# TritonDataCenter/dragnet

Measured on NVIDIA B200. Metric: json_records_per_sec, higher is better.
Workload: dtype u8

## Files before the change

dragnet_b200/csrc/api.cu:

```cuda
#include <cuda_runtime.h>
#include <dlfcn.h>
#include <fcntl.h>
#include <sys/stat.h>
#include <unistd.h>

#include <algorithm>
#include <map>
#include <condition_variable>
#include <mutex>
#include <thread>
#include <cerrno>
#include <cmath>
#include <cstdio>
#include <cstdlib>
#include <cstring>
#include <string>
#include <vector>

#include "../../include/dragnet_gpu.h"
#include "plan.h"
#include "result.h"
#include "scan_kernel.cuh"
#include "fast_kernel.cuh"
#include "jit.h"
// ... 114 lines not shown
	size_t ring_cap = 0;
	u8 *d_ring[RING_SLOTS] = {};
	u8 *h_stage[RING_SLOTS] = {};
	cudaEvent_t ev_ready[RING_SLOTS] = {}, ev_free[RING_SLOTS] = {};
	bool slot_used[RING_SLOTS] = {};
	size_t next_slot = 0;
	u8 *d_carry = nullptr;
	size_t carry_len = 0;
	u8 *d_side = nullptr;
	u8 *file_buf = nullptr;
	cudaEvent_t file_done[32] = {};
	std::vector<std::pair<cudaEvent_t, cudaEvent_t>> ev_pairs;
	std::vector<cudaEvent_t> ev_pool;
	double kernel_ms = 0;
	uint64_t launches = 0, kernel_bytes = 0, bytes_fed = 0;
	uint64_t aux_launches = 0;
	cudaEvent_t ev_init = nullptr;
	bool finished = false;
	bool tmpl_enabled = true, tmpl_tried = false;
	bool warp_kernel = false;
	u32 wslice = DNG_W_SLICE_MAX;
	int kernel_pref = 0;
	u32 w_sslots = 0, w_s1slots = 0;
	unsigned long long *h_live = nullptr;
	unsigned long long learn_lines = 0, learn_tmpl = 0;
	unsigned long long seen_lines = 0, seen_long = 0;
	int relearns = 0;
	u8 *d_tmpl = nullptr;
	u32 tmpl_bytes = 0, ntemplates = 0;
	FPlan fplan;
	FPlan *d_fplan = nullptr;
	u8 *d_ftmpl = nullptr;
	u32 ftmpl_bytes = 0, nftemplates = 0, ftmpl_leaf_off = 0, ftmpl_pool_off = 0;
	bool f_kernel = false;
	u32 f_nt = DNG_F_NT;
	unsigned long long seen_over = 0, seen_aggr = 0;
	bool f_probed = false;
	u32 f_nsl = 13;
	double mean_line = 224;
	u32 f_smem_max = 0;
	int jit_mode = 1;
	std::shared_ptr<JitKernels> jit;
	uint64_t jit_launches = 0;
	MissEnt *d_miss = nullptr;
	u32 *d_miss_n = nullptr;
	u32 miss_cap = 0;
	unsigned long long seen_tmpl = 0;
	std::string err;
	int err_code = 0;

	int fail(int code, const std::string &m) {
		if (!err_code) {
			err_code = code;
			err = m;
		}
		return code;
	}
	int cuda(cudaError_t e, const char *what) {
		if (e == cudaSuccess)
			return 0;
		return fail(DNG_ECUDA, std::string(what) + ": " +
		    cudaGetErrorString(e));
	}
};

#define CK(s, call) do { if ((s)->cuda((call), #call)) return (s)->err_code; } while (0)
// ... 17 lines not shown
__global__ void resolve_pairs_kernel(const DevPlan *plan, const u8 *lines,
    const u32 *se, u32 n, TResolved *out)
{
	u32 i = blockIdx.x * blockDim.x + threadIdx.x;
	if (i >= n)
		return;
	RecState R;
	parse_record(lines + se[2 * i], se[2 * i + 1] - se[2 * i], *plan, R);
	out[i].flags = R.flags;
	out[i].set_mask = R.set_mask;
	for (int k = 0; k < MAX_SLOTS; k++)
		out[i].slots[k] = ((R.set_mask >> k) & 1) ? R.slots[k] : 0;
}

static std::mutex g_fnt_mu;
static std::map<unsigned long long, u32> g_fnt_memo;

static unsigned long long fplan_hash(const FPlan &F)
{
	unsigned long long h = 1469598103934665603ull;
	const u8 *p = (const u8 *)&F;
	for (size_t i = 0; i < sizeof (F); i++)
		h = (h ^ p[i]) * 1099511628211ull;
	return h;
}

static void fnt_remember(const dng_scan *s)
{
	std::lock_guard<std::mutex> g(g_fnt_mu);
	g_fnt_memo[fplan_hash(s->fplan)] = s->f_nt;
}

int learn_ftemplates(dng_scan *s, const std::vector<TCandidate> &cands,
    const std::vector<TResolved> &res, size_t sampled_lines)
{
	std::vector<TResolved> fres(res.size());
	for (size_t i = 0; i < res.size(); i++)
		fplan_resolve(s->plan.dev, res[i], fres[i]);
	std::vector<u8> blob, accepted;
	u32 nt = 0;
	tmpl_build(cands, fres, TMPL_RESERVE, blob, &nt, true, &accepted);
	cached_free(s->d_ftmpl);
	s->d_ftmpl = nullptr;
	s->ftmpl_bytes = 0;
	s->nftemplates = 0;
	if (!blob.empty()) {
		const THdr *th = (const THdr *)blob.data();
		s->ftmpl_leaf_off = th->leaf_off;
		s->ftmpl_pool_off = th->pool_off;
	}
	size_t covered = 0;
	for (size_t i = 0; i < cands.size(); i++)
		if (accepted[i])
			covered += cands[i].count;
	if (!blob.empty()) {
		size_t padded = (blob.size() + 127) & ~(size_t)127;
		blob.resize(padded, 0);
		CK(s, DEV_ALLOC(s, &s->d_ftmpl, padded));
		CK(s, cudaMemcpyAsync(s->d_ftmpl, blob.data(), padded,
		    cudaMemcpyHostToDevice, s->stream));
		CK(s, cudaStreamSynchronize(s->stream));
		s->ftmpl_bytes = (u32)padded;
		s->nftemplates = nt;
	}
	s->jit.reset();
	if (s->jit_mode && !blob.empty())
		s->jit = jit_request(jit_source(blob.data(), blob.size(), &s->fplan),
		    (int)s->f_nsl, s->device, (int)s->f_smem_max,
		    s->jit_mode == 2);
	if (s->kernel_pref == 0)
		s->f_kernel = s->warp_kernel && !blob.empty() &&
		    covered * 10 >= sampled_lines * 9 &&
		    s->mean_line * DNG_F_NLCAP >= 32.0 * 16 * s->f_nsl * 1.5;
	return 0;
}

int learn_templates(dng_scan *s, const u8 *data, unsigned long long start,
    unsigned long long nbytes)
{
	s->tmpl_tried = true;
	if (!s->tmpl_enabled && s->kernel_pref != 0)
		return 0;
	size_t n = (size_t)std::min<unsigned long long>(nbytes - start,
	    TMPL_SAMPLE_BYTES);
	u8 *hbuf = nullptr;
	CK(s, HOST_ALLOC(&hbuf, TMPL_SAMPLE_BYTES));
	struct Release {
		u8 *p;
		~Release() { cached_free(p); }
	} release{hbuf};
	CK(s, cudaMemcpyAsync(hbuf, data + start, n, cudaMemcpyDeviceToHost,
	    s->stream));
	CK(s, cudaStreamSynchronize(s->stream));
	struct { u8 *p; u8 *data() const { return p; }
	    u8 operator[](size_t i) const { return p[i]; } } head{hbuf};
	if (s->kernel_pref == 0) {
		size_t longest = 0, run = 0;
		for (size_t i = 0; i < n; i++) {
			if (head[i] == '\n') {
				longest = std::max(longest, run);
				run = 0;
			} else {
// ... 53 lines not shown
	    (size_t)TMPL_MAX_LEAVES * (TMPL_MAX_LINE + 1) + 16);
	if (e == cudaSuccess)
		e = DEV_ALLOC(s, &d_offs, 2 * (TMPL_MAX_LEAVES + 1) * sizeof (u32));
	if (e == cudaSuccess)
		e = DEV_ALLOC(s, &d_res, TMPL_MAX_LEAVES * sizeof (TResolved));
	if (e == cudaSuccess)
		e = cudaMemcpyAsync(d_lines, lines.data(), lines.size(),
		    cudaMemcpyHostToDevice, s->stream);
	std::vector<u32> se;
	for (size_t i = 0; i < cands.size(); i++) {
		se.push_back(offs[i]);
		se.push_back(offs[i + 1] - 1);
	}
	if (e == cudaSuccess)
		e = cudaMemcpyAsync(d_offs, se.data(), se.size() * sizeof (u32),
		    cudaMemcpyHostToDevice, s->stream);
	if (e == cudaSuccess) {
		s->aux_launches++;
		resolve_pairs_kernel<<<1, 32, 0, s->stream>>>(s->d_plan, d_lines,
		    d_offs, (u32)cands.size(), d_res);
		e = cudaGetLastError();
	}
	if (e == cudaSuccess)
		e = cudaMemcpyAsync(res.data(), d_res,
		    res.size() * sizeof (TResolved), cudaMemcpyDeviceToHost,
		    s->stream);
	if (e == cudaSuccess)
		e = cudaStreamSynchronize(s->stream);
	cached_free(d_lines);
	cached_free(d_offs);
	cached_free(d_res);
	if (e != cudaSuccess)
		return s->cuda(e, "template resolve");
	if (s->fplan.ok && learn_ftemplates(s, cands, res, sampled_lines))
		return s->err_code;
	std::vector<u8> blob;
	u32 nt = 0;
	tmpl_build(cands, res, TMPL_RESERVE, blob, &nt);
	if (blob.empty())
		return 0;
	size_t padded = (blob.size() + 127) & ~(size_t)127;
	blob.resize(padded, 0);
	cached_free(s->d_tmpl);
	s->d_tmpl = nullptr;
	s->tmpl_bytes = 0;
	CK(s, DEV_ALLOC(s, &s->d_tmpl, padded));
	CK(s, cudaMemcpyAsync(s->d_tmpl, blob.data(), padded,
	    cudaMemcpyHostToDevice, s->stream));
	CK(s, cudaStreamSynchronize(s->stream));
	s->tmpl_bytes = (u32)padded;
	s->ntemplates = nt;
	return 0;
}

template <int NSL>
void launch_fkernel(dng_scan *s, const FScanArgs &a, u32 grid)
{
	scan_kernel_f<NSL><<<grid, s->f_nt, fkernel_smem<NSL>(a.tmpl_bytes,
	    a.s1slots, a.sslots, a.nrows, s->f_nt / 32), s->stream>>>(a);
}

template <int NSL>
void fkernel_slots(const dng_scan *s, u32 nrows, u32 tmpl_room, u32 *s1, u32 *s2)
{
	const size_t fixed = fkernel_smem<NSL>(tmpl_room, 0, 0, nrows,
	    s->f_nt / 32);
	const size_t room = s->f_smem_max > fixed ? s->f_smem_max - fixed : 0;
	u32 n1 = 32;
	while (n1 < 1024 && (size_t)n1 * 2 * sizeof (SSlot1) +
	    DNG_SSLOTS_MIN * sizeof (SSlot) <= room * 3 / 4)
		n1 *= 2;
	const size_t left = room - std::min(room, (size_t)n1 * sizeof (SSlot1));
	u32 n2 = DNG_SSLOTS_MIN;
	while (n2 * 2 <= DNG_SSLOTS_MAX && (size_t)n2 * 2 * sizeof (SSlot) <= left)
		n2 *= 2;
	*s1 = n1;
	*s2 = n2;
}

int launch_fscan(dng_scan *s, const u8 *data, unsigned long long start,
    unsigned long long nbytes, bool final)
{
	if (!s->d_miss) {
		s->miss_cap = (u32)env_size("DNG_MISS_CAP", (size_t)4 << 20);
		CK(s, DEV_ALLOC(s, &s->d_miss, (size_t)s->miss_cap *
		    sizeof (MissEnt)));
		CK(s, DEV_ALLOC(s, &s->d_miss_n, 64));
		CK(s, cudaMemsetAsync(s->d_miss_n, 0, 64, s->stream));
	}
	const unsigned long long skip = start & ~15ull;
	data += skip;
	start -= skip;
	nbytes -= skip;
	FScanArgs a;
	a.data = data;
	a.start = start;
	a.nbytes = nbytes;
	a.fplan = s->d_fplan;
	a.plan = s->d_plan;
	a.tmpl = s->d_ftmpl;
	a.tmpl_bytes = s->ftmpl_bytes;
	a.leaf_off = s->ftmpl_leaf_off;
	a.pool_off = s->ftmpl_pool_off;
	a.counters = s->d_counters;
	a.tab = s->tab;
	a.final = final ? 1 : 0;
	a.nrows = s->fplan.nrows;
	a.miss = s->d_miss;
	a.miss_cap = s->miss_cap;
	a.miss_n = s->d_miss_n;
	const u32 nsl = s->f_nsl;
	const unsigned long long chunk = 32ull * 16 * nsl;
	a.nchunks = (u32)((nbytes + chunk - 1) / chunk);
	const u32 nw = s->f_nt / 32;
	const u32 grid = std::min<u32>((a.nchunks + nw - 1) / nw,
	    (u32)s->sm_count);
	const u32 nwarps = grid * nw;
	a.seg = std::max<u32>(1, std::min<u32>(DNG_F_SEG,
	    a.nchunks / (nwarps * 8)));
	a.seg_next = s->d_miss_n + 1;
	cudaMemsetAsync(s->d_miss_n, 0, 2 * sizeof (u32), s->stream);
	cudaEvent_t e0 = get_event(s), e1 = get_event(s);
	cudaEventRecord(e0, s->stream);
	const bool jit = s->jit && s->jit->state.load() == 1 && s->ftmpl_bytes;
	const u32 tmpl_room = jit ? 0 : (u32)TMPL_RESERVE;
	if (jit)
		a.tmpl_bytes = 0;
	size_t smem = 0;
	switch (nsl) {
	case 7:
		fkernel_slots<7>(s, a.nrows, tmpl_room, &a.s1slots, &a.sslots);
		smem = fkernel_smem<7>(a.tmpl_bytes, a.s1slots, a.sslots, a.nrows,
		    s->f_nt / 32);
		if (!jit)
			launch_fkernel<7>(s, a, grid);
		break;
	case 9:
		fkernel_slots<9>(s, a.nrows, tmpl_room, &a.s1slots, &a.sslots);
		smem = fkernel_smem<9>(a.tmpl_bytes, a.s1slots, a.sslots, a.nrows,
		    s->f_nt / 32);
		if (!jit)
			launch_fkernel<9>(s, a, grid);
		break;
	case 11:
		fkernel_slots<11>(s, a.nrows, tmpl_room, &a.s1slots, &a.sslots);
		smem = fkernel_smem<11>(a.tmpl_bytes, a.s1slots, a.sslots, a.nrows,
		    s->f_nt / 32);
		if (!jit)
			launch_fkernel<11>(s, a, grid);
		break;
	default:
		fkernel_slots<13>(s, a.nrows, tmpl_room, &a.s1slots, &a.sslots);
		smem = fkernel_smem<13>(a.tmpl_bytes, a.s1slots, a.sslots, a.nrows,
		    s->f_nt / 32);
		if (!jit)
			launch_fkernel<13>(s, a, grid);
		break;
	}
	cudaError_t le = cudaSuccess;
	if (jit) {
		void *args[] = { &a };
		le = cudaLaunchKernel((const void *)s->jit->kern, dim3(grid),
		    dim3(s->f_nt), args, smem, s->stream);
		s->jit_launches++;
	}
	if (le == cudaSuccess)
		le = cudaGetLastError();
	FMissArgs ma;
	ma.data = data;
	ma.start = start;
	ma.plan = s->d_plan;
	ma.plan_bytes = s->plan_bytes;
	ma.counters = s->d_counters;
	ma.tab = s->tab;
	ma.s1slots = 64;
	ma.sslots = 1024;
	ma.miss = s->d_miss;
	ma.miss_n = s->d_miss_n;
	ma.miss_cap = s->miss_cap;
	if (le == cudaSuccess) {
		scan_miss_kernel<<<s->sm_count * 2, DNG_MISS_NT, s->plan_bytes +
		    ma.s1slots * sizeof (SSlot1) + ma.sslots * sizeof (SSlot),
		    s->stream>>>(ma);
		le = cudaGetLastError();
	}
	cudaEventRecord(e1, s->stream);
	if (!s->h_live && HOST_ALLOC(&s->h_live, NCTR * sizeof (unsigned long long))
// ... 1069 lines not shown
	if (!s)
		return;
	cudaSetDevice(s->device);
	if (s->stream)
		cudaStreamSynchronize(s->stream);
	if (s->own_stream && s->own_stream != s->stream)
		cudaStreamSynchronize(s->own_stream);
	if (s->copy_stream)
		cudaStreamSynchronize(s->copy_stream);
	drain_events(s);
	if (s->ev_init)
		cudaEventDestroy(s->ev_init);
	for (auto e : s->ev_pool)
		cudaEventDestroy(e);
	for (size_t i = 0; i < RING_SLOTS; i++) {
		if (s->d_ring[i]) {
			cached_free(s->d_ring[i]);
			cudaEventDestroy(s->ev_ready[i]);
			cudaEventDestroy(s->ev_free[i]);
		}
		if (s->h_stage[i])
			cached_free(s->h_stage[i]);
	}
	if (s->file_buf) {
		cached_free(s->file_buf);
		for (int i = 0; i < 32; i++)
			cudaEventDestroy(s->file_done[i]);
	}
	cached_free(s->h_live);
	cached_free(s->d_plan);
	cached_free(s->d_tmpl);
	cached_free(s->d_fplan);
	cached_free(s->d_ftmpl);
	cached_free(s->d_miss);
	cached_free(s->d_miss_n);
	cached_free(s->tab.entries);
	cached_free(s->tab.arena);
	cached_free(s->tab.misc);
	cached_free(s->d_counters);
	cached_free(s->d_nl);
	cached_free(s->d_carry);
	cached_free(s->d_side);
	if (s->own_stream)
		cudaStreamDestroy(s->own_stream);
	if (s->copy_stream)
		cudaStreamDestroy(s->copy_stream);
	delete s;
}

void *dng_pinned_alloc(size_t len)
{
	void *p = nullptr;
	if (cudaMallocHost(&p, len) != cudaSuccess)
		return nullptr;
	return p;
}

void dng_pinned_free(void *p)
{
	if (p)
		cudaFreeHost(p);
}


size_t dng_result_count(const dng_result *r)
{
// ... 188 lines not shown
```

dragnet_b200/csrc/fast.cuh:

```cuda
#ifndef DNG_FAST_CUH
#define DNG_FAST_CUH

#include "fast.h"
#include "tmpl.cuh"

#ifdef DNG_JIT_HOT
#define DNG_PLAN_LOOP _Pragma("unroll")
#else
#define DNG_PLAN_LOOP _Pragma("unroll 1")
#endif

namespace dng {

#include "fscan.cuh"

DNG_HD u32 fcap_off(u32 c) { return c & 0xfff; }
DNG_HD u32 fcap_len(u32 c) { return (c >> 12) & 0xfff; }
DNG_HD u32 fcap_type(u32 c) { return (c >> 24) & 7; }
DNG_HD u32 fcap_flag(u32 c) { return c >> 27; }

template <class M>
DNG_HD bool fmatch(M &m, u32 len, bool active, u32 &defmask)
{
	u32 p = 0;
// ... 461 lines not shown
		if (n > 1)
			first |= fpiece_byte(m, F, pc, 1) << 24;
		const u32 fm = n >= 2 ? ~0u : n == 1 ? 0x00ffffffu : 0x0000ffffu;
		diff |= (kc.next() ^ first) & fm;
		if (n > 2) {
			if (pc.kind == 0) {
				FWords<M> ws(m, F, pc, 2);
				const u32 r = n - 2;
#pragma unroll 1
				for (u32 i = 0; i < r; i += 4) {
					const u32 mk = i + 4 <= r ? ~0u :
					    (1u << (8 * (r & 3))) - 1;
					diff |= (kc.next() ^ ws.next()) & mk;
				}
			} else {
				const u32 r = n - 2;
#pragma unroll 1
				for (u32 i = 0; i < r; i += 4) {
					u32 w = 0;
					for (u32 x = 0; x < 4 && i + x < r; x++)
						w |= fpiece_byte(m, F, pc, 2 + i + x)
						    << (8 * x);
					const u32 mk = i + 4 <= r ? ~0u :
					    (1u << (8 * (r & 3))) - 1;
					diff |= (kc.next() ^ w) & mk;
				}
			}
		}
		o += 2 + n;
	}
	return diff == 0;
}

template <class M>
DNG_HD void fkey_write(M &m, const FPlan &F, u32 defmask, u8 *out)
{
	u32 o = 0;
DNG_PLAN_LOOP
	for (u32 j = 0; j < F.ncols; j++) {
		FPiece pc;
		fpiece(m, F, j, defmask, pc);
		if (pc.kind == 2) {
			out[o] = 0xff;
			out[o + 1] = 0xff;
			for (u32 k = 0; k < 4; k++) {
				out[o + 2 + k] = (u8)(pc.lo >> (8 * k));
				out[o + 6 + k] = (u8)(pc.hi >> (8 * k));
			}
			o += 10;
			continue;
		}
		out[o] = (u8)pc.n;
		out[o + 1] = (u8)(pc.n >> 8);
#pragma unroll 1
		for (u32 k = 0; k < pc.n; k++)
			out[o + 2 + k] = (u8)fpiece_byte(m, F, pc, k);
		o += 2 + pc.n;
	}
	while (o & 7)
		out[o++] = 0;
}

#ifndef __CUDACC__
struct FastHostMem : TmplHostMem {
	u32 caps[F_MAXROWS];
	const u8 *ptr(u32 off) const { return rec + off; }
	u32 litw(u32 off) const { return pool32(off); }
	void setcap(u32 p, u32 v) { caps[p] = v; }
	u32 getcap(u32 p) const { return caps[p]; }
};
struct FastHostKey {
	const u8 *key;
	u32 len;
	struct Cur {
		const FastHostKey *k;
		u32 off;
		u32 next() {
			u32 w = 0;
			for (u32 x = 0; x < 4; x++)
				if (off + x < k->len)
					w |= (u32)k->key[off + x] << (8 * x);
			off += 4;
			return w;
		}
	};
	Cur cursor(u32 off) const { Cur c; c.k = this; c.off = off; return c; }
};
#endif

}
#endif
```

dragnet_b200/csrc/fast.h:

```cpp
#ifndef DNG_FAST_H
#define DNG_FAST_H

#include "plan.h"
#include "tmpl.h"

namespace dng {

enum : int {
	F_MAXPATHS = 8, F_MAXCODE = 16, F_MAXCOLS = 6, F_MAXSYN = 2,
	F_POOL = 512, F_MAXKEY = 256,
	F_MAXLINE = 4095,
	F_MAXROWS = F_MAXPATHS + 2 * F_MAXCOLS,
	F_NT = 896
};

enum : u16 { FC_UNDEFINED = 0, FC_NULL = 12, FC_TRUE = 16, FC_FALSE = 20,
	FC_END = 28 };

struct alignas(16) FPlan {
	Leaf code[F_MAXCODE];
	Col col[F_MAXCOLS];
	u8 syn_path[F_MAXSYN];
	int16_t ds_entry, user_entry, time_entry;
	u8 nsyn, ncols, npaths, ok;
	u8 ord_row[F_MAXCOLS];
	u8 nrows;
	u8 ncode;
	u8 pad[4];
	char pool[F_POOL];
};

#define DNG_FCAP(type, off, len, flag) \
	((u32)(off) | ((u32)(len) << 12) | ((u32)(type) << 24) | ((u32)(flag) << 27))

enum : u32 {
	FO_AGGR = 0, FO_MISS, FO_DS_FILTERED, FO_DS_FAILED, FO_USER_FILTERED,
	FO_USER_FAILED, FO_SYNTH_UNDEF, FO_SYNTH_BADDATE, FO_TIME_FILTERED,
	FO_TIME_FAILED
};

}

#include <vector>

namespace dng {

void fplan_build(const DevPlan &P, FPlan &F);

bool fplan_resolve(const DevPlan &P, const TResolved &in, TResolved &out);

}

#endif
```

dragnet_b200/csrc/fast_jit_cold.cu:

```cuda
#define DNG_NO_GENERAL_KERNELS
#include "fast_kernel.cuh"

using namespace dng;

extern "C" __device__ void dng_cold_slow_add(FSmem m, const FPlan *F,
    u32 defmask, u32 klen, STab stab, const GTable *gt)
{
	fslow_add(m, F, defmask, klen, stab, gt);
}

extern "C" __device__ void dng_cold_miss(const u8 *data,
    unsigned long long start, unsigned long long beg, unsigned long long end,
    const DevPlan *plan, STab stab, const GTable *gt,
    unsigned long long *counters)
{
	fmiss_inline(data, start, beg, end, plan, stab, gt, counters);
}

extern "C" __device__ void dng_cold_flush(STab stab, u32 s1slots, u32 sslots,
    const GTable *tab)
{
	flush_tally(stab, s1slots, sslots, *tab);
}
```

dragnet_b200/csrc/fast_kernel.cuh:

```cuda
#ifndef DNG_FAST_KERNEL_CUH
#define DNG_FAST_KERNEL_CUH

#include <stddef.h>

#include "scan_kernel.cuh"
#include "fast.cuh"

namespace dng {

#define DNG_F_NT F_NT
#define DNG_F_NW (DNG_F_NT / 32)
#define DNG_F_PRE 512
#define DNG_F_SLACK 64
#define DNG_F_NLCAP 128
#define DNG_F_MAXLINE DNG_F_PRE
#define DNG_F_SEG 16

struct MissEnt {
	unsigned long long beg;
	unsigned long long end;
};

struct FScanArgs {
	const u8 *data;
	unsigned long long start;
	unsigned long long nbytes;
	const FPlan *fplan;
	const DevPlan *plan;
	const u8 *tmpl;
	u32 tmpl_bytes;
	u32 leaf_off, pool_off;
	unsigned long long *counters;
	GTable tab;
	u32 nchunks, seg;
	u32 final;
	u32 s1slots, sslots;
	u32 nrows;
	MissEnt *miss;
	u32 miss_cap;
	u32 *miss_n;
	u32 *seg_next;
};

template <int NSL>
struct FWarpSmem {
	static constexpr u32 CHUNK = 32 * 16 * NSL;
	static constexpr u32 BUF = DNG_F_PRE + CHUNK + DNG_F_SLACK;
	static constexpr u32 BYTES = (BUF + 2 * DNG_F_NLCAP + 16 + 127) & ~127u;
};

static constexpr u32 FPLAN_SMEM = (sizeof (FPlan) + 127) & ~127u;

template <int NSL>
static inline size_t fkernel_smem(u32 tmpl_bytes, u32 s1slots, u32 sslots,
    u32 nrows, u32 nw = DNG_F_NW)
{
	return FPLAN_SMEM + tmpl_bytes + (size_t)s1slots * sizeof (SSlot1) +
	    (size_t)sslots * sizeof (SSlot) + (size_t)nrows * DNG_F_NT * 4 +
	    (size_t)nw * FWarpSmem<NSL>::BYTES;
}

__device__ __forceinline__ void mbar_init_sa(u32 bar, u32 count)
{
	asm volatile("mbarrier.init.shared::cta.b64 [%0], %1;"
	    :: "r"(bar), "r"(count) : "memory");
	asm volatile("fence.mbarrier_init.release.cluster;" ::: "memory");
}

__device__ __forceinline__ void mbar_expect_tx_sa(u32 bar, u32 bytes)
{
	asm volatile("mbarrier.arrive.expect_tx.shared::cta.b64 _, [%0], %1;"
	    :: "r"(bar), "r"(bytes) : "memory");
}

__device__ __forceinline__ void tma_load_1d_sa(u32 dst, const void *src,
    u32 bytes, u32 bar)
{
	asm volatile("cp.async.bulk.shared::cluster.global.mbarrier::"
	    "complete_tx::bytes [%0], [%1], %2, [%3];"
	    :: "r"(dst), "l"(src), "r"(bytes), "r"(bar) : "memory");
}

__device__ __forceinline__ void mbar_wait_sa(u32 bar, u32 parity)
{
	asm volatile(
	    "{\n"
	    ".reg .pred p;\n"
	    "WAIT_%=:\n"
	    "mbarrier.try_wait.parity.shared::cta.b64 p, [%0], %1;\n"
	    "@p bra DONE_%=;\n"
	    "bra WAIT_%=;\n"
	    "DONE_%=:\n"
// ... 83 lines not shown
	{
		sts32(caps + p * (DNG_F_NT * 4), v);
	}
	__device__ __forceinline__ u32 getcap(u32 p) const
	{
		return lds32(caps + p * (DNG_F_NT * 4));
	}
};

struct FKeySmem {
	u32 ka;
	typedef TmplSmem::Cur Cur;
	__device__ __forceinline__ Cur cursor(u32 off) const
	{
		Cur c;
		const u32 a = ka + off;
		c.sh = (a & 3) * 8;
		c.wa = (a & ~3u) + 4;
		c.w0 = lds32(c.wa - 4);
		c.w1 = lds32(c.wa);
		return c;
	}
};

#ifdef DNG_JIT_HOT
extern "C" __device__ void dng_cold_slow_add(FSmem m, const FPlan *F,
    u32 defmask, u32 klen, STab stab, const GTable *gt);
extern "C" __device__ void dng_cold_miss(const u8 *data,
    unsigned long long start, unsigned long long beg, unsigned long long end,
    const DevPlan *plan, STab stab, const GTable *gt,
    unsigned long long *counters);
extern "C" __device__ void dng_cold_flush(STab stab, u32 s1slots, u32 sslots,
    const GTable *tab);
extern "C" __constant__ const FPlan dng_jplan;
#define fslow_add dng_cold_slow_add
#define fmiss_inline dng_cold_miss
#else
__device__ __noinline__ void fslow_add(FSmem m, const FPlan *F, u32 defmask,
    u32 klen, STab stab, const GTable *gt)
{
	__align__(8) u8 kbuf[F_MAXKEY + 16];
	fkey_write(m, *F, defmask, kbuf);
	const unsigned long long *kw = (const unsigned long long *)kbuf;
	shared_add(stab, *gt, key_hash_words(kw, klen), kw, klen, 1);
}

#endif

__device__ __forceinline__ unsigned long long lds64_acquire(u32 addr)
{
	unsigned long long v;
	asm volatile("ld.acquire.cta.shared.u64 %0, [%1];" : "=l"(v) : "r"(addr)
	    : "memory");
	return v;
}

__device__ __forceinline__ void sts64_release(u32 addr, unsigned long long v)
{
	asm volatile("st.release.cta.shared.u64 [%0], %1;" :: "r"(addr), "l"(v)
	    : "memory");
}

__device__ __forceinline__ void ftally(FSmem &m, const FPlan &F,
    const FPlan *Fcold, u32 defmask, u32 h, u32 klen, const STab &stab,
    const GTable &gt, u32 over_sa)
{
	if (klen <= DNG_SKEY) {
// ... 76 lines not shown
	if (at < a.miss_cap) {
		MissEnt e;
		e.beg = beg;
		e.end = end;
		a.miss[at] = e;
	} else {
		fmiss_inline(a.data, a.start, beg, end, a.plan, stab, &a.tab,
		    a.counters);
	}
}

extern "C" __device__ unsigned dng_jmatch(unsigned ra, unsigned len,
    unsigned active, unsigned caps);

template <int NSL, bool JIT>
__device__ __forceinline__ void fscan_body(const FScanArgs &a)
{
	typedef FWarpSmem<NSL> WS;
	constexpr u32 CHUNK = WS::CHUNK, SLICE = 16 * NSL, D0 = DNG_F_PRE;
	extern __shared__ __align__(128) u8 smem[];
#ifdef DNG_JIT_HOT
	const FPlan &F = dng_jplan;
#else
	const FPlan &F = *(const FPlan *)smem;
#endif
	u8 *sp = smem + FPLAN_SMEM;
	const u32 tmpl_sa = smem_u32(sp);
	sp += a.tmpl_bytes;
	STab stab;
	stab.s1 = (SSlot1 *)sp;
	sp += a.s1slots * sizeof (SSlot1);
	stab.s = (SSlot *)sp;
	sp += a.sslots * sizeof (SSlot);
	stab.mask1 = a.s1slots - 1;
	stab.mask = a.sslots - 1;
	const u32 caps_sa = smem_u32(sp);
	sp += a.nrows * DNG_F_NT * 4;

	const u32 tid = threadIdx.x;
	const u32 lane = tid & 31, wid = tid >> 5;
	const u32 sb = smem_u32(sp) + wid * WS::BYTES;
	const u32 nlpos = sb + WS::BUF;
	const u32 mbar = sb + WS::BUF + 2 * DNG_F_NLCAP;

	{
		const uint4 *src = (const uint4 *)a.fplan;
		uint4 *dst = (uint4 *)smem;
		for (u32 i = tid; i < FPLAN_SMEM / 16; i += blockDim.x)
			dst[i] = src[i];
		const uint4 *tsrc = (const uint4 *)a.tmpl;
		uint4 *tdst = (uint4 *)(smem + FPLAN_SMEM);
		for (u32 i = tid; i < a.tmpl_bytes / 16; i += blockDim.x)
			tdst[i] = tsrc[i];
		const uint4 z = make_uint4(0, 0, 0, 0);
		uint4 *tz = (uint4 *)stab.s1;
		const u32 tab_bytes = a.s1slots * (u32)sizeof (SSlot1) +
		    a.sslots * (u32)sizeof (SSlot);
		for (u32 i = tid; i < tab_bytes / 16; i += blockDim.x)
			tz[i] = z;
		if (lane == 0)
			mbar_init_sa(mbar, 1);
		if (lane < DNG_F_SLACK / 4)
			sts32(sb + D0 + CHUNK + 4 * lane, 0x22222222u);
	}
	__syncthreads();

	const bool use_tmpl = a.tmpl_bytes != 0;
	FSmem m;
	m.ra = 0;
	m.nodes = tmpl_sa + (u32)sizeof (THdr);
	m.leaves = tmpl_sa + a.leaf_off;
	m.pool = tmpl_sa + a.pool_off;
	m.caps = caps_sa + tid * 4;

	__shared__ u32 s_drop[16];
	if (tid < 16)
		s_drop[tid] = 0;
	u32 ntmpl = 0, naggr = 0, parity = 0;
	const u32 ltmask = (1u << lane) - 1;

	const u32 nwarps = gridDim.x * (blockDim.x >> 5);
	const u32 gw = wid * gridDim.x + blockIdx.x;
	const u32 nseg = (a.nchunks + a.seg - 1) / a.seg;

	for (u32 seg = gw; seg < nseg; ) {
		const u32 ch0 = seg * a.seg;
		const u32 ch1 = min(ch0 + a.seg, a.nchunks);
		int beg0 = 0;
		unsigned long long open_abs = ~0ull;
		for (u32 ch = ch0; ch < ch1; ch++) {
// ... 151 lines not shown
									    pos);
							}
						}
					}
				}
				__syncwarp();

				for (u32 rb = 0; rb < total; rb += 32) {
					const u32 r = rb + lane;
					const bool have = r < total;
					int beg = 0;
					u32 end = 0;
					if (have) {
						end = lds16(nlpos + 2 * r);
						beg = r ? (int)lds16(nlpos + 2 * r - 2) + 1 :
						    beg0;
					}
					const bool inbuf = have && beg >= 0 &&
					    end - (u32)beg <= F_MAXLINE;
					const u32 len = inbuf ? end - (u32)beg : 0;
					m.ra = sb + (inbuf ? (u32)beg : 0);
					u32 defmask = 0;
					u32 fo = FO_MISS;
					bool matched;
					if (JIT) {
						const u32 r_ = dng_jmatch(m.ra, len, inbuf,
						    m.caps);
						matched = r_ & 1;
						defmask = r_ >> 1;
					} else {
						matched = use_tmpl &&
						    fmatch(m, len, inbuf, defmask);
					}
					if (matched) {
						double s0, s1;
						fo = fstage(m, F, defmask, s0, s1);
						u32 h = 0, klen = 0, slow = 0;
						if (fo == FO_AGGR && (!fprep(m, F, defmask,
						    s0, s1, slow) || !fkey_hash(m, F,
						    defmask, h, klen)))
							fo = FO_MISS;
						if (fo == FO_AGGR) {
							if (slow)
								atomicAdd(&s_drop[1], 1u);
							ftally(m, F, (const FPlan *)smem, defmask,
							    h, klen, stab, a.tab,
							    smem_u32(&s_drop[15]));
						}
					}
					const bool done = fo != FO_MISS;
					ntmpl += __popc(__ballot_sync(0xffffffffu, done));
					naggr += __popc(__ballot_sync(0xffffffffu,
					    fo == FO_AGGR));
					{
						u32 dm = __ballot_sync(0xffffffffu,
						    fo >= FO_DS_FILTERED);
						while (dm) {
							const u32 f0 = __shfl_sync(0xffffffffu,
							    fo, __ffs(dm) - 1);
							const u32 same = __ballot_sync(
							    0xffffffffu, fo == f0);
							if (lane == 0)
								atomicAdd(&s_drop[f0],
								    (u32)__popc(same));
							dm &= ~same;
						}
					}
					const bool miss = have && !done;
					const u32 mm = __ballot_sync(0xffffffffu, miss);
					if (mm) {
						u32 base = 0;
						if (lane == 0)
							base = atomicAdd(a.miss_n,
							    (u32)__popc(mm));
						base = __shfl_sync(0xffffffffu, base, 0);
						if (miss)
							fmiss_put(a, stab, base +
							    __popc(mm & ltmask), r ? g0 - D0 +
							    (u32)beg : open_abs, g0 - D0 + end);
					}
				}
				__syncwarp();
				const u32 lastnl = lds16(nlpos + 2 * (total - 1));
				beg0 = (int)lastnl + 1;
				open_abs = g0 - D0 + lastnl + 1;
				__syncwarp();
			}
			if (vnl && lane == 0) {
				fmiss_put(a, stab, atomicAdd(a.miss_n, 1u), open_abs,
				    a.nbytes);
			}
			beg0 -= (int)CHUNK;
			if (beg0 < 0)
				beg0 = -1;
		}
		if (lane == 0)
			seg = nwarps + atomicAdd(a.seg_next, 1u);
		seg = __shfl_sync(0xffffffffu, seg, 0);
	}

#ifdef DNG_JIT_HOT
	__syncthreads();
	dng_cold_flush(stab, a.s1slots, a.sslots, &a.tab);
#else
	flush_tally(stab, a.s1slots, a.sslots, a.tab);
#endif
	if (lane == 0) {
		if (ntmpl) {
			atomicAdd(&a.counters[CTR_LINES], (unsigned long long)ntmpl);
			atomicAdd(&a.counters[CTR_TMPL], (unsigned long long)ntmpl);
		}
		if (naggr)
			atomicAdd(&a.counters[CTR_AGGR], (unsigned long long)naggr);
	}
	if (tid == 15 && s_drop[15])
		atomicAdd(&a.counters[CTR_OVER], (unsigned long long)s_drop[15]);
	if (tid < 15 && s_drop[tid]) {
		const int ctr = tid == 1 ? (int)CTR_SLOW :
		    tid == FO_DS_FILTERED ? (int)CTR_DS_FILTERED :
		    tid == FO_DS_FAILED ? (int)CTR_DS_FAILED :
		    tid == FO_USER_FILTERED ? (int)CTR_USER_FILTERED :
		    tid == FO_USER_FAILED ? (int)CTR_USER_FAILED :
		    tid == FO_SYNTH_UNDEF ? (int)CTR_SYNTH_UNDEF :
		    tid == FO_SYNTH_BADDATE ? (int)CTR_SYNTH_BADDATE :
		    tid == FO_TIME_FILTERED ? (int)CTR_TIME_FILTERED :
		    tid == FO_TIME_FAILED ? (int)CTR_TIME_FAILED : -1;
		if (ctr >= 0)
			atomicAdd(&a.counters[ctr], (unsigned long long)s_drop[tid]);
	}
}

#ifndef DNG_JIT_HOT
template <int NSL>
__global__ void __launch_bounds__(DNG_F_NT, 1)
scan_kernel_f(const FScanArgs a)
// ... 82 lines not shown
```

dragnet_b200/csrc/jit.cpp:

```cpp
#include <dlfcn.h>
#include <stdarg.h>
#include <stdio.h>
#include <stdlib.h>
#include <string.h>

#include <chrono>
#include <functional>
#include <map>
#include <mutex>
#include <set>
#include <vector>

#include "jit.h"
#include "fast.h"
#include "tmpl.h"

#define BLOB(n) extern "C" const unsigned char n[]; \
	extern "C" const unsigned char n##_end[];
BLOB(dng_jit_hot7) BLOB(dng_jit_hot9) BLOB(dng_jit_hot11) BLOB(dng_jit_hot13)
BLOB(dng_jit_cold)
#undef BLOB
extern "C" const char dng_fscan_src[];
extern "C" const char dng_fscan_src_end[];

// ... 145 lines not shown
	for (int i = 0; i < F_MAXCODE; i++) {
		const Leaf &l = F.code[i];
		u64 cb;
		memcpy(&cb, &l.cnum, 8);
		appendf(s, "		{ 0x%016llxull, %u, %u, %d, %d, %u, %u, { %u, %u }, 0 },\n",
		    (unsigned long long)cb, (unsigned)l.coff, (unsigned)l.clen, (int)l.jt,
		    (int)l.jf, (unsigned)l.op, (unsigned)l.cstr,
		    (unsigned)l.src.kind, (unsigned)l.src.idx);
	}
	s += "	},\n	{\n";
	for (int i = 0; i < F_MAXCOLS; i++) {
		const Col &c = F.col[i];
		u64 sb;
		memcpy(&sb, &c.step, 8);
		appendf(s, "		{ 0x%016llxull, { %u, %u }, %u, { 0, 0, 0, 0, 0 } },\n",
		    (unsigned long long)sb, (unsigned)c.src.kind, (unsigned)c.src.idx,
		    (unsigned)c.kind);
	}
	appendf(s, "	},\n	{ %u, %u }, %d, %d, %d, %u, %u, %u, %u,\n",
	    (unsigned)F.syn_path[0], (unsigned)F.syn_path[1], (int)F.ds_entry,
	    (int)F.user_entry, (int)F.time_entry, (unsigned)F.nsyn,
	    (unsigned)F.ncols, (unsigned)F.npaths, (unsigned)F.ok);
	appendf(s, "	{ %u, %u, %u, %u, %u, %u }, %u, %u, { 0, 0, 0, 0 },\n	{ ",
	    (unsigned)F.ord_row[0], (unsigned)F.ord_row[1],
	    (unsigned)F.ord_row[2], (unsigned)F.ord_row[3],
	    (unsigned)F.ord_row[4], (unsigned)F.ord_row[5], (unsigned)F.nrows,
	    (unsigned)F.ncode);
	for (int i = 0; i < F_POOL; i++)
		appendf(s, "%d,%s", (int)(signed char)F.pool[i],
		    i % 32 == 31 ? "\n	  " : "");
	s += " }\n};\n";
}

std::string jit_source(const u8 *blob, size_t bytes, const FPlan *plan,
    const char *prelude)
{
	std::string s;
	s += "/* generated by libdragnet_gpu (jit.cpp) */\n";
	bool shared = plan && plan->ncols >= 3;
	if (const char *sh = getenv("DNG_JIT_SHARED"))
		shared = atoi(sh) == 1;
	if (!prelude && shared)
		s += "#define DNG_JIT_SHARED_SCAN\n";
	s += prelude ? prelude : PRELUDE;
	if (plan)
		plan_source(*plan, s);
	s.append(dng_fscan_src, (size_t)(dng_fscan_src_end - dng_fscan_src));
	s += "\nextern \"C\" __device__ unsigned dng_jmatch(unsigned ra, "
	    "unsigned len, unsigned active, unsigned caps)\n{\n"
	    "	JMem m;\n	m.ra = ra;\n"
	    "	u32 p = 0, q = 0, val = 0, dm = 0, res = 0;\n";
	if (bytes < sizeof (THdr)) {
		s += "	return 0;\n}\n";
		return s;
	}
	THdr h;
	memcpy(&h, blob, sizeof (h));
	const TNode *tn = (const TNode *)(blob + sizeof (THdr));
	const u8 *pool = blob + h.pool_off;
	auto pool32 = [&](u32 off) {
		u32 v;
		memcpy(&v, pool + off, 4);
		return v;
	};
	const u32 N = h.nnodes;
	std::vector<JN> nd(N);
	bool str_takes_quote = false;
	for (u32 i = 0; i < N; i++) {
		const TNode &t = tn[i];
		JN &n = nd[i];
		n.lit.assign((const char *)pool + t.lit, t.len);
		n.kind = t.kind;
		n.cap = t.cap;
		n.leaf = (t.next & TN_LEAF) != 0;
		n.leaf_mask = 0;
		if (n.leaf)
			memcpy(&n.leaf_mask, blob + h.leaf_off +
			    4 * (t.next & 0x7fff), 4);
		n.next = n.leaf ? -1 : (int)t.next;
		n.alt = t.alt == TN_NOALT ? -1 : (int)t.alt;
// ... 443 lines not shown
```

dragnet_b200/csrc/jit.h:

```cpp
#ifndef DNG_JIT_H
#define DNG_JIT_H

#include <cuda_runtime.h>

#include <atomic>
#include <memory>
#include <string>

#include "fast.h"

namespace dng {

struct JitKernels {
	cudaLibrary_t lib = nullptr;
	cudaKernel_t kern = nullptr;
	std::atomic<int> state{0};
	bool ok = false;
	std::string err;
	double compile_ms = 0, link_ms = 0;
};

std::string jit_source(const u8 *blob, size_t bytes, const FPlan *plan,
    const char *prelude = nullptr);

std::shared_ptr<JitKernels> jit_request(const std::string &source, int nsl,
    int dev, int smem_max, bool wait);

bool jit_prepare();

bool jit_build(const std::string &source, int nsl, std::string &cubin,
    std::string &err, double *compile_ms, double *link_ms);

}

#endif
```

Before: 9.599 billion.

## Add dense dictionary counters for low-cardinality discrete group keys in JIT kernel

Learns, on the host, a small dictionary of the most frequent values for each discrete path column from a sample of records. When these values cover nearly all records, it generates JIT code that maps each record's columns straight to a dense index by comparing against literal words. The kernel then increments a per-block shared-memory counter array instead of hashing the key and probing the tally hash table. At the end each block flushes its nonzero dense counters to the global table, optionally first merging duplicate codes within a warp via match_any. This adds shared memory use, fallback paths for values outside the dictionary, and extra JIT codegen complexity.

```diff
diff --git a/dragnet_b200/csrc/api.cu b/dragnet_b200/csrc/api.cu
--- a/dragnet_b200/csrc/api.cu
+++ b/dragnet_b200/csrc/api.cu
@@ -170,6 +170,8 @@
 	FPlan *d_fplan = nullptr;
 	u8 *d_ftmpl = nullptr;
 	u32 ftmpl_bytes = 0, nftemplates = 0, ftmpl_leaf_off = 0, ftmpl_pool_off = 0;
+	FDict fdict{};
+	FDict *d_fdict = nullptr;
 	bool f_kernel = false;
 	u32 f_nt = DNG_F_NT;
 	unsigned long long seen_over = 0, seen_aggr = 0;
@@ -253,7 +255,8 @@
 }
 
 int learn_ftemplates(dng_scan *s, const std::vector<TCandidate> &cands,
-    const std::vector<TResolved> &res, size_t sampled_lines)
+    const std::vector<TResolved> &res, size_t sampled_lines, const u8 *head,
+    size_t nhead)
 {
 	std::vector<TResolved> fres(res.size());
 	for (size_t i = 0; i < res.size(); i++)
@@ -274,21 +277,30 @@
 	for (size_t i = 0; i < cands.size(); i++)
 		if (accepted[i])
 			covered += cands[i].count;
+	memset(&s->fdict, 0, sizeof (s->fdict));
+	if (s->jit_mode && !blob.empty() && jit_dense())
+		fdict_learn(s->fplan, blob.data(), head, nhead, s->fdict);
 	if (!blob.empty()) {
 		size_t padded = (blob.size() + 127) & ~(size_t)127;
 		blob.resize(padded, 0);
 		CK(s, DEV_ALLOC(s, &s->d_ftmpl, padded));
 		CK(s, cudaMemcpyAsync(s->d_ftmpl, blob.data(), padded,
 		    cudaMemcpyHostToDevice, s->stream));
+		if (s->fdict.ncols) {
+			if (!s->d_fdict)
+				CK(s, DEV_ALLOC(s, &s->d_fdict, sizeof (FDict)));
+			CK(s, cudaMemcpyAsync(s->d_fdict, &s->fdict,
+			    sizeof (FDict), cudaMemcpyHostToDevice, s->stream));
+		}
 		CK(s, cudaStreamSynchronize(s->stream));
 		s->ftmpl_bytes = (u32)padded;
 		s->nftemplates = nt;
 	}
 	s->jit.reset();
 	if (s->jit_mode && !blob.empty())
-		s->jit = jit_request(jit_source(blob.data(), blob.size(), &s->fplan),
-		    (int)s->f_nsl, s->device, (int)s->f_smem_max,
-		    s->jit_mode == 2);
+		s->jit = jit_request(jit_source(blob.data(), blob.size(), &s->fplan,
+		    nullptr, &s->fdict), (int)s->f_nsl, s->device,
+		    (int)s->f_smem_max, s->jit_mode == 2);
 	if (s->kernel_pref == 0)
 		s->f_kernel = s->warp_kernel && !blob.empty() &&
 		    covered * 10 >= sampled_lines * 9 &&
@@ -408,7 +420,8 @@
 	cached_free(d_res);
 	if (e != cudaSuccess)
 		return s->cuda(e, "template resolve");
-	if (s->fplan.ok && learn_ftemplates(s, cands, res, sampled_lines))
+	if (s->fplan.ok && learn_ftemplates(s, cands, res, sampled_lines,
+	    head.data(), n))
 		return s->err_code;
 	std::vector<u8> blob;
 	u32 nt = 0;
@@ -433,14 +446,16 @@
 void launch_fkernel(dng_scan *s, const FScanArgs &a, u32 grid)
 {
 	scan_kernel_f<NSL><<<grid, s->f_nt, fkernel_smem<NSL>(a.tmpl_bytes,
-	    a.s1slots, a.sslots, a.nrows, s->f_nt / 32), s->stream>>>(a);
+	    a.s1slots, a.sslots, a.nrows, s->f_nt / 32, a.ndense),
+	    s->stream>>>(a);
 }
 
 template <int NSL>
-void fkernel_slots(const dng_scan *s, u32 nrows, u32 tmpl_room, u32 *s1, u32 *s2)
+void fkernel_slots(const dng_scan *s, u32 nrows, u32 tmpl_room, u32 ndense,
+    u32 *s1, u32 *s2)
 {
 	const size_t fixed = fkernel_smem<NSL>(tmpl_room, 0, 0, nrows,
-	    s->f_nt / 32);
+	    s->f_nt / 32, ndense);
 	const size_t room = s->f_smem_max > fixed ? s->f_smem_max - fixed : 0;
 	u32 n1 = 32;
 	while (n1 < 1024 && (size_t)n1 * 2 * sizeof (SSlot1) +
@@ -502,33 +517,39 @@
 	const u32 tmpl_room = jit ? 0 : (u32)TMPL_RESERVE;
 	if (jit)
 		a.tmpl_bytes = 0;
+	a.ndense = jit && s->fdict.ncols ? (s->fdict.total + 3) & ~3u : 0;
+	a.dict = a.ndense ? s->d_fdict : nullptr;
 	size_t smem = 0;
 	switch (nsl) {
 	case 7:
-		fkernel_slots<7>(s, a.nrows, tmpl_room, &a.s1slots, &a.sslots);
+		fkernel_slots<7>(s, a.nrows, tmpl_room, a.ndense, &a.s1slots,
+		    &a.sslots);
 		smem = fkernel_smem<7>(a.tmpl_bytes, a.s1slots, a.sslots, a.nrows,
-		    s->f_nt / 32);
+		    s->f_nt / 32, a.ndense);
 		if (!jit)
 			launch_fkernel<7>(s, a, grid);
 		break;
 	case 9:
-		fkernel_slots<9>(s, a.nrows, tmpl_room, &a.s1slots, &a.sslots);
+		fkernel_slots<9>(s, a.nrows, tmpl_room, a.ndense, &a.s1slots,
+		    &a.sslots);
 		smem = fkernel_smem<9>(a.tmpl_bytes, a.s1slots, a.sslots, a.nrows,
-		    s->f_nt / 32);
+		    s->f_nt / 32, a.ndense);
 		if (!jit)
 			launch_fkernel<9>(s, a, grid);
 		break;
 	case 11:
-		fkernel_slots<11>(s, a.nrows, tmpl_room, &a.s1slots, &a.sslots);
+		fkernel_slots<11>(s, a.nrows, tmpl_room, a.ndense, &a.s1slots,
+		    &a.sslots);
 		smem = fkernel_smem<11>(a.tmpl_bytes, a.s1slots, a.sslots, a.nrows,
-		    s->f_nt / 32);
+		    s->f_nt / 32, a.ndense);
 		if (!jit)
 			launch_fkernel<11>(s, a, grid);
 		break;
 	default:
-		fkernel_slots<13>(s, a.nrows, tmpl_room, &a.s1slots, &a.sslots);
+		fkernel_slots<13>(s, a.nrows, tmpl_room, a.ndense, &a.s1slots,
+		    &a.sslots);
 		smem = fkernel_smem<13>(a.tmpl_bytes, a.s1slots, a.sslots, a.nrows,
-		    s->f_nt / 32);
+		    s->f_nt / 32, a.ndense);
 		if (!jit)
 			launch_fkernel<13>(s, a, grid);
 		break;
@@ -1664,6 +1685,7 @@
 	cached_free(s->d_tmpl);
 	cached_free(s->d_fplan);
 	cached_free(s->d_ftmpl);
+	cached_free(s->d_fdict);
 	cached_free(s->d_miss);
 	cached_free(s->d_miss_n);
 	cached_free(s->tab.entries);
diff --git a/dragnet_b200/csrc/fast.cuh b/dragnet_b200/csrc/fast.cuh
--- a/dragnet_b200/csrc/fast.cuh
+++ b/dragnet_b200/csrc/fast.cuh
@@ -517,6 +517,31 @@
 	return diff == 0;
 }
 
+template <class B>
+DNG_HD u32 fkey_put(u8 *out, u32 o, u32 n, const B &byte)
+{
+	out[o] = (u8)n;
+	out[o + 1] = (u8)(n >> 8);
+#pragma unroll 1
+	for (u32 k = 0; k < n; k++)
+		out[o + 2 + k] = (u8)byte(k);
+	return o + 2 + n;
+}
+
+DNG_HD void fkey_pad(u8 *out, u32 o)
+{
+	while (o & 7)
+		out[o++] = 0;
+}
+
+template <class M>
+struct FPieceBytes {
+	M *m;
+	const FPlan *F;
+	const FPiece *pc;
+	DNG_HD u32 operator()(u32 k) const { return fpiece_byte(*m, *F, *pc, k); }
+};
+
 template <class M>
 DNG_HD void fkey_write(M &m, const FPlan &F, u32 defmask, u8 *out)
 {
@@ -535,15 +560,31 @@
 			o += 10;
 			continue;
 		}
-		out[o] = (u8)pc.n;
-		out[o + 1] = (u8)(pc.n >> 8);
-#pragma unroll 1
-		for (u32 k = 0; k < pc.n; k++)
-			out[o + 2 + k] = (u8)fpiece_byte(m, F, pc, k);
-		o += 2 + pc.n;
-	}
-	while (o & 7)
-		out[o++] = 0;
+		FPieceBytes<M> b;
+		b.m = &m;
+		b.F = &F;
+		b.pc = &pc;
+		o = fkey_put(out, o, pc.n, b);
+	}
+	fkey_pad(out, o);
+}
+
+struct FDictBytes {
+	const u8 *v;
+	DNG_HD u32 operator()(u32 k) const { return v[k]; }
+};
+
+DNG_HD u32 fdense_key(const FDict &D, u32 idx, u8 *out)
+{
+	u32 o = 0;
+	for (u32 j = 0; j < D.ncols; j++) {
+		const u32 c = idx / D.stride[j] % D.n[j];
+		FDictBytes b;
+		b.v = D.val[j][c];
+		o = fkey_put(out, o, D.len[j][c], b);
+	}
+	fkey_pad(out, o);
+	return o;
 }
 
 #ifndef __CUDACC__
diff --git a/dragnet_b200/csrc/fast.h b/dragnet_b200/csrc/fast.h
--- a/dragnet_b200/csrc/fast.h
+++ b/dragnet_b200/csrc/fast.h
@@ -30,6 +30,18 @@
 	char pool[F_POOL];
 };
 
+enum : int { F_DICT_VALS = 15, F_DICT_BYTES = 24, F_DENSE_MAX = 1024 };
+
+struct alignas(16) FDict {
+	u32 ncols;
+	u32 total;
+	u32 n[F_MAXCOLS];
+	u32 stride[F_MAXCOLS];
+	u8 path[F_MAXCOLS];
+	u8 len[F_MAXCOLS][F_DICT_VALS];
+	u8 val[F_MAXCOLS][F_DICT_VALS][F_DICT_BYTES];
+};
+
 #define DNG_FCAP(type, off, len, flag) \
 	((u32)(off) | ((u32)(len) << 12) | ((u32)(type) << 24) | ((u32)(flag) << 27))
 
@@ -49,6 +61,9 @@
 
 bool fplan_resolve(const DevPlan &P, const TResolved &in, TResolved &out);
 
+bool fdict_learn(const FPlan &F, const u8 *blob, const u8 *head, size_t n,
+    FDict &D);
+
 }
 
 #endif
diff --git a/dragnet_b200/csrc/fast_jit_cold.cu b/dragnet_b200/csrc/fast_jit_cold.cu
--- a/dragnet_b200/csrc/fast_jit_cold.cu
+++ b/dragnet_b200/csrc/fast_jit_cold.cu
@@ -22,3 +22,29 @@
 {
 	flush_tally(stab, s1slots, sslots, *tab);
 }
+
+extern "C" __device__ u32 dng_cold_key(FSmem m, const FPlan *F, u32 defmask,
+    STab stab, const GTable *gt, u32 over_sa)
+{
+	u32 h, klen;
+	if (!fkey_hash(m, *F, defmask, h, klen))
+		return 0;
+	ftally(m, *F, F, defmask, h, klen, stab, *gt, over_sa);
+	return 1;
+}
+
+extern "C" __device__ void dng_cold_dense_flush(u32 dense_sa, const FDict *D,
+    const GTable *gt)
+{
+	const u32 total = D->total;
+	for (u32 i = threadIdx.x; i < total; i += blockDim.x) {
+		const u32 c = lds32(dense_sa + 4 * i);
+		if (!c)
+			continue;
+		__align__(8) u8 kbuf[F_MAXKEY + 16];
+		const u32 klen = fdense_key(*D, i, kbuf);
+		const unsigned long long *kw = (const unsigned long long *)kbuf;
+		global_add(*gt, key_hash_words(kw, klen), kbuf, klen,
+		    (unsigned long long)c);
+	}
+}
diff --git a/dragnet_b200/csrc/fast_kernel.cuh b/dragnet_b200/csrc/fast_kernel.cuh
--- a/dragnet_b200/csrc/fast_kernel.cuh
+++ b/dragnet_b200/csrc/fast_kernel.cuh
@@ -35,6 +35,8 @@
 	u32 nchunks, seg;
 	u32 final;
 	u32 s1slots, sslots;
+	u32 ndense;
+	const FDict *dict;
 	u32 nrows;
 	MissEnt *miss;
 	u32 miss_cap;
@@ -53,11 +55,11 @@
 
 template <int NSL>
 static inline size_t fkernel_smem(u32 tmpl_bytes, u32 s1slots, u32 sslots,
-    u32 nrows, u32 nw = DNG_F_NW)
+    u32 nrows, u32 nw = DNG_F_NW, u32 ndense = 0)
 {
 	return FPLAN_SMEM + tmpl_bytes + (size_t)s1slots * sizeof (SSlot1) +
-	    (size_t)sslots * sizeof (SSlot) + (size_t)nrows * DNG_F_NT * 4 +
-	    (size_t)nw * FWarpSmem<NSL>::BYTES;
+	    (size_t)sslots * sizeof (SSlot) + (size_t)ndense * 4 +
+	    (size_t)nrows * DNG_F_NT * 4 + (size_t)nw * FWarpSmem<NSL>::BYTES;
 }
 
 __device__ __forceinline__ void mbar_init_sa(u32 bar, u32 count)
@@ -207,7 +209,14 @@
     unsigned long long *counters);
 extern "C" __device__ void dng_cold_flush(STab stab, u32 s1slots, u32 sslots,
     const GTable *tab);
+extern "C" __device__ u32 dng_cold_key(FSmem m, const FPlan *F, u32 defmask,
+    STab stab, const GTable *gt, u32 over_sa);
+extern "C" __device__ void dng_cold_dense_flush(u32 dense_sa, const FDict *D,
+    const GTable *gt);
 extern "C" __constant__ const FPlan dng_jplan;
+extern "C" __constant__ const unsigned dng_jdense;
+extern "C" __device__ unsigned dng_jcode(unsigned ra, unsigned dm,
+    unsigned caps);
 #define fslow_add dng_cold_slow_add
 #define fmiss_inline dng_cold_miss
 #else
@@ -350,6 +359,8 @@
 	sp += a.s1slots * sizeof (SSlot1);
 	stab.s = (SSlot *)sp;
 	sp += a.sslots * sizeof (SSlot);
+	const u32 dense_sa = smem_u32(sp);
+	sp += a.ndense * 4;
 	stab.mask1 = a.s1slots - 1;
 	stab.mask = a.sslots - 1;
 	const u32 caps_sa = smem_u32(sp);
@@ -373,7 +384,7 @@
 		const uint4 z = make_uint4(0, 0, 0, 0);
 		uint4 *tz = (uint4 *)stab.s1;
 		const u32 tab_bytes = a.s1slots * (u32)sizeof (SSlot1) +
-		    a.sslots * (u32)sizeof (SSlot);
+		    a.sslots * (u32)sizeof (SSlot) + a.ndense * 4;
 		for (u32 i = tid; i < tab_bytes / 16; i += blockDim.x)
 			tz[i] = z;
 		if (lane == 0)
@@ -591,22 +602,51 @@
 						matched = use_tmpl &&
 						    fmatch(m, len, inbuf, defmask);
 					}
+					u32 dc = ~0u;
 					if (matched) {
 						double s0, s1;
 						fo = fstage(m, F, defmask, s0, s1);
 						u32 h = 0, klen = 0, slow = 0;
-						if (fo == FO_AGGR && (!fprep(m, F, defmask,
-						    s0, s1, slow) || !fkey_hash(m, F,
-						    defmask, h, klen)))
+						if (fo == FO_AGGR && !fprep(m, F, defmask,
+						    s0, s1, slow))
 							fo = FO_MISS;
+#ifdef DNG_JIT_HOT
+						if (fo == FO_AGGR && (dng_jdense & 1))
+							dc = dng_jcode(m.ra, defmask, m.caps);
+						if (dc != ~0u) {
+						} else if (fo == FO_AGGR &&
+						    (dng_jdense & 3) == 1) {
+							if (!dng_cold_key(m, (const FPlan *)smem,
+							    defmask, stab, &a.tab,
+							    smem_u32(&s_drop[15])))
+								fo = FO_MISS;
+						} else
+#endif
 						if (fo == FO_AGGR) {
-							if (slow)
-								atomicAdd(&s_drop[1], 1u);
-							ftally(m, F, (const FPlan *)smem, defmask,
-							    h, klen, stab, a.tab,
-							    smem_u32(&s_drop[15]));
+							if (!fkey_hash(m, F, defmask, h, klen))
+								fo = FO_MISS;
+							else
+								ftally(m, F, (const FPlan *)smem,
+								    defmask, h, klen, stab, a.tab,
+								    smem_u32(&s_drop[15]));
 						}
-					}
+						if (fo == FO_AGGR && slow)
+							atomicAdd(&s_drop[1], 1u);
+					}
+#ifdef DNG_JIT_HOT
+					if (dng_jdense & 4) {
+						const u32 peers = __match_any_sync(
+						    0xffffffffu, dc);
+						if (dc != ~0u && !(peers & ltmask))
+							asm volatile("red.shared.add.u32 "
+							    "[%0], %1;" :: "r"(dense_sa +
+							    4 * dc), "r"(__popc(peers))
+							    : "memory");
+					} else if (dc != ~0u) {
+						asm volatile("red.shared.add.u32 [%0], 1;"
+						    :: "r"(dense_sa + 4 * dc) : "memory");
+					}
+#endif
 					const bool done = fo != FO_MISS;
 					ntmpl += __popc(__ballot_sync(0xffffffffu, done));
 					naggr += __popc(__ballot_sync(0xffffffffu,
@@ -660,6 +700,8 @@
 
 #ifdef DNG_JIT_HOT
 	__syncthreads();
+	if (a.ndense)
+		dng_cold_dense_flush(dense_sa, a.dict, &a.tab);
 	dng_cold_flush(stab, a.s1slots, a.sslots, &a.tab);
 #else
 	flush_tally(stab, a.s1slots, a.sslots, a.tab);
diff --git a/dragnet_b200/csrc/fdict.cpp b/dragnet_b200/csrc/fdict.cpp
--- /dev/null
+++ b/dragnet_b200/csrc/fdict.cpp
@@ -0,0 +1,115 @@
+#include <string.h>
+
+#include <algorithm>
+#include <map>
+#include <string>
+#include <vector>
+
+#include "fast.cuh"
+
+namespace dng {
+
+namespace {
+
+constexpr size_t DICT_SAMPLE_BYTES = 16 * 1024;
+
+}
+
+bool fdict_learn(const FPlan &F, const u8 *blob, const u8 *head, size_t n,
+    FDict &D)
+{
+	memset(&D, 0, sizeof (D));
+	if (!F.ok || F.ncols == 0 || !blob)
+		return false;
+	for (u32 j = 0; j < F.ncols; j++)
+		if (F.col[j].kind != COL_DISCRETE || F.col[j].src.kind != SRC_PATH)
+			return false;
+	n = std::min(n, DICT_SAMPLE_BYTES);
+	const u32 nc = F.ncols;
+	std::vector<std::map<std::string, u32>> freq(nc);
+	std::vector<std::string> recs;
+	size_t nrec = 0;
+	size_t pos = 0;
+	while (pos < n) {
+		const u8 *nl = (const u8 *)memchr(head + pos, '\n', n - pos);
+		if (!nl)
+			break;
+		const size_t end = (size_t)(nl - head);
+		const u32 len = (u32)(end - pos);
+		const u8 *rec = head + pos;
+		pos = end + 1;
+		if (len > F_MAXLINE)
+			continue;
+		FastHostMem fm;
+		fm.rec = rec;
+		fm.len = len;
+		fm.blob = blob;
+		u32 defmask = 0, slow = 0;
+		double s0 = 0, s1 = 0;
+		if (!fmatch(fm, len, true, defmask) ||
+		    fstage(fm, F, defmask, s0, s1) != FO_AGGR ||
+		    !fprep(fm, F, defmask, s0, s1, slow))
+			continue;
+		nrec++;
+		for (u32 j = 0; j < nc; j++) {
+			FPiece pc;
+			fpiece(fm, F, j, defmask, pc);
+			const char *b = pc.kind == 0 ? (const char *)rec + pc.off :
+			    F.pool + pc.off;
+			std::string v(b, pc.n);
+			freq[j][v]++;
+			recs.push_back(v);
+		}
+	}
+	if (nrec == 0)
+		return false;
+	std::vector<std::vector<std::string>> vals(nc);
+	u32 total = 1;
+	for (u32 j = 0; j < nc; j++) {
+		std::vector<std::pair<u32, std::string>> byf;
+		for (auto &kv : freq[j])
+			if (kv.first.size() <= (size_t)F_DICT_BYTES)
+				byf.push_back(std::make_pair(kv.second, kv.first));
+		std::sort(byf.begin(), byf.end(), [](const std::pair<u32,
+		    std::string> &a, const std::pair<u32, std::string> &b) {
+			return a.first != b.first ? a.first > b.first :
+			    a.second < b.second;
+		});
+		if (byf.size() > (size_t)F_DICT_VALS)
+			byf.resize(F_DICT_VALS);
+		for (auto &p : byf)
+			vals[j].push_back(p.second);
+		std::sort(vals[j].begin(), vals[j].end());
+		if (vals[j].empty())
+			return false;
+		total *= (u32)vals[j].size();
+		if (total > (u32)F_DENSE_MAX)
+			return false;
+	}
+	size_t covered = 0;
+	for (size_t r = 0; r < nrec; r++) {
+		bool in = true;
+		for (u32 j = 0; j < nc && in; j++)
+			in = std::binary_search(vals[j].begin(), vals[j].end(),
+			    recs[r * nc + j]);
+		covered += in;
+	}
+	if (covered * 100 < nrec * 99)
+		return false;
+	D.ncols = nc;
+	D.total = total;
+	u32 stride = 1;
+	for (int j = (int)nc - 1; j >= 0; j--) {
+		D.n[j] = (u32)vals[j].size();
+		D.stride[j] = stride;
+		D.path[j] = F.col[j].src.idx;
+		stride *= D.n[j];
+		for (u32 c = 0; c < D.n[j]; c++) {
+			D.len[j][c] = (u8)vals[j][c].size();
+			memcpy(D.val[j][c], vals[j][c].data(), vals[j][c].size());
+		}
+	}
+	return true;
+}
+
+}
diff --git a/dragnet_b200/csrc/jit.cpp b/dragnet_b200/csrc/jit.cpp
--- a/dragnet_b200/csrc/jit.cpp
+++ b/dragnet_b200/csrc/jit.cpp
@@ -201,8 +201,77 @@
 	s += " }\n};\n";
 }
 
+unsigned jit_dense()
+{
+	const char *v = getenv("DNG_DENSE");
+	return v ? (unsigned)atoi(v) : 1u;
+}
+
+static void dense_source(const FDict &D, std::string &s)
+{
+	s += "extern \"C\" __device__ unsigned dng_jcode(unsigned ra, unsigned dm, "
+	    "unsigned caps)\n{\n	JMem m;\n	m.ra = ra;\n	u32 idx = 0;\n";
+	for (u32 j = 0; j < D.ncols; j++) {
+		const u32 p = D.path[j];
+		appendf(s, "	{	/* column %u: path %u, %u values */\n", j, p,
+		    D.n[j]);
+		appendf(s, "	const u32 cw = (dm >> %uu) & 1u ? jlds32(caps + %uu) "
+		    ": 0u;\n", p, p * (u32)F_NT * 4u);
+		s += "	const u32 t = (cw >> 24) & 7u, n = (cw >> 12) & 0xfffu;\n"
+		    "	u32 c = 0xffffffffu;\n"
+		    "	if (t == T_STR || t == T_NUM) {\n"
+		    "		JMem::Cur k = m.cursor(cw & 0xfffu);\n"
+		    "		switch (n) {\n";
+		std::map<u32, std::vector<u32>> bylen;
+		for (u32 c = 0; c < D.n[j]; c++)
+			bylen[D.len[j][c]].push_back(c);
+		for (auto &bl : bylen) {
+			const u32 L = bl.first, nw = (L + 3) / 4;
+			appendf(s, "		case %u: {\n", L);
+			for (u32 w = 0; w < nw; w++) {
+				if (w + 1 == nw && (L & 3))
+					appendf(s, "			const u32 w%u = k.next() & "
+					    "0x%08xu;\n", w, (1u << (8 * (L & 3))) - 1);
+				else
+					appendf(s, "			const u32 w%u = k.next();\n",
+					    w);
+			}
+			bool first = true;
+			for (u32 c : bl.second) {
+				s += first ? "			if (" : "			else if (";
+				first = false;
+				if (nw == 0)
+					s += "true";
+				for (u32 w = 0; w < nw; w++) {
+					u32 lit = 0;
+					for (u32 x = 0; x < 4 && 4 * w + x < L; x++)
+						lit |= (u32)D.val[j][c][4 * w + x] <<
+						    (8 * x);
+					appendf(s, "%sw%u == 0x%08xu", w ? " && " : "",
+					    w, lit);
+				}
+				appendf(s, ")\n				c = %uu;\n",
+				    c * D.stride[j]);
+			}
+			s += "			break;\n		}\n";
+		}
+		s += "		}\n	}\n";
+		static const struct { u32 t; const char *v; } K[] = {
+			{ T_UNDEF, "undefined" }, { T_NULL, "null" },
+			{ T_TRUE, "true" }, { T_FALSE, "false" } };
+		for (auto &kc : K)
+			for (u32 c = 0; c < D.n[j]; c++)
+				if (D.len[j][c] == strlen(kc.v) &&
+				    !memcmp(D.val[j][c], kc.v, D.len[j][c]))
+					appendf(s, "	if (t == %uu)\n		c = %uu;\n",
+					    kc.t, c * D.stride[j]);
+		s += "	if (c == 0xffffffffu)\n		return c;\n	idx += c;\n	}\n";
+	}
+	s += "	return idx;\n}\n";
+}
+
 std::string jit_source(const u8 *blob, size_t bytes, const FPlan *plan,
-    const char *prelude)
+    const char *prelude, const FDict *dict)
 {
 	std::string s;
 	s += "/* generated by libdragnet_gpu (jit.cpp) */\n";
@@ -215,6 +284,16 @@
 	if (plan)
 		plan_source(*plan, s);
 	s.append(dng_fscan_src, (size_t)(dng_fscan_src_end - dng_fscan_src));
+	const unsigned mode = jit_dense();
+	const bool dense = dict && dict->ncols && mode;
+	if (plan)
+		appendf(s, "\nextern \"C\" __constant__ const unsigned dng_jdense = "
+		    "%uu;\n", dense ? mode | 1u : 0u);
+	if (dense)
+		dense_source(*dict, s);
+	else if (plan)
+		s += "extern \"C\" __device__ unsigned dng_jcode(unsigned, unsigned, "
+		    "unsigned)\n{\n	return 0xffffffffu;\n}\n";
 	s += "\nextern \"C\" __device__ unsigned dng_jmatch(unsigned ra, "
 	    "unsigned len, unsigned active, unsigned caps)\n{\n"
 	    "	JMem m;\n	m.ra = ra;\n"
diff --git a/dragnet_b200/csrc/jit.h b/dragnet_b200/csrc/jit.h
--- a/dragnet_b200/csrc/jit.h
+++ b/dragnet_b200/csrc/jit.h
@@ -21,7 +21,9 @@
 };
 
 std::string jit_source(const u8 *blob, size_t bytes, const FPlan *plan,
-    const char *prelude = nullptr);
+    const char *prelude = nullptr, const FDict *dict = nullptr);
+
+unsigned jit_dense();
 
 std::shared_ptr<JitKernels> jit_request(const std::string &source, int nsl,
     int dev, int smem_max, bool wait);
```

After: 10.45 billion (median of 6 runs). 8.9% higher.
